# SamsungLabs/fcaf3d

Measured on AMD Instinct MI355X. Metric: scenes/sec fwd+bwd, ScanNet 100k-pt 2cm voxels, 1/2/4/8 MI355X, higher is better.
Workload: dtype f32

## Files before the change

### fcaf3d_amd/csrc/conv.hip

```cpp
#include "fc_common.h"
#include "../../include/fcaf3d_hip.h"
#ifdef FC_TRACE
__device__ unsigned long long* g_trace_buf_lds;
__device__ int g_trace_cap_lds;
extern "C" int fc_debug_trace_lds(unsigned long long* buf, int cap) {
  FC_HIP(hipMemcpyToSymbol(HIP_SYMBOL(g_trace_buf_lds), &buf, sizeof(buf)));
  FC_HIP(hipMemcpyToSymbol(HIP_SYMBOL(g_trace_cap_lds), &cap, sizeof(cap)));
  return FC_OK;
}
#define TR_BUF g_trace_buf_lds
#define TR_CAP g_trace_cap_lds
#endif
#include "fc_trace.h"

typedef float f32x16 __attribute__((ext_vector_type(16)));
typedef float f32x2 __attribute__((ext_vector_type(2)));
typedef float f32x4 __attribute__((ext_vector_type(4)));

__device__ __attribute__((aligned(16))) float g_zero_row[64];

__device__ int g_fc_prio;
extern "C" int fc_debug_set_prio(int mode) {
  FC_HIP(hipMemcpyToSymbol(HIP_SYMBOL(g_fc_prio), &mode, sizeof(mode)));
  return FC_OK;
// ... 1220 lines not shown
    else if (r.bm == 128) FC_TILE(128, 64, 2);
    else if (r.bn == 128) launch_conv_fp32<64, 128, 2>(r, a, grid);
    else launch_conv_fp32<64, 64, 2>(r, a, grid);
#undef FC_TILE
  }
  FC_CHECK_LAUNCH();
  return FC_OK;
}
#undef FC_LAUNCH
#undef FC_LAUNCH_EPI

extern "C" {

int fc_conv_fwd_route(int64_t n_in, int64_t n_out, int K, int Cin, int Cout, int flags, int table_kind, int64_t live_tiles, int* out) {
  if (!out || n_in < 0 || n_out < 0 || K < 1 || Cin < 1 || Cout < 1) return FC_EINVAL;
  const ConvRoute r = conv_route({n_in, n_out, K, Cin, Cout}, flags, table_kind, live_tiles, route_env());
  const int f[16] = {r.family, r.bm, r.bn, r.wm, r.S, r.wsrc, r.mode, r.buf, r.epi, (int)r.grid[0], (int)r.grid[1], (int)r.grid[2]};
  for (int i = 0; i < 16; ++i) out[i] = f[i];
  return r.family == FC_FAM_INVALID ? FC_EINVAL : FC_OK;
}

int64_t fc_conv_fwd_ws_bytes(int64_t n_out, int K, int Cin, int Cout, int flags) {
  const ConvRoute r = conv_route({n_out, n_out, K, Cin, Cout}, flags, FC_TABLE_DENSE, 0, route_env());
  return r.S > 1 ? (int64_t)r.S * n_out * Cout * (int64_t)sizeof(float) : 0;
}

int64_t fc_conv_fwd_pairs_ws_bytes(int64_t n_out, int K, int Cout) {
  return (int64_t)K * n_out * Cout * (int64_t)sizeof(float);
}

int64_t fc_conv_stats_blocks(int64_t n_out, int K, int Cin, int Cout, int flags, int pairs) {
  if (n_out < 1) return 0;
  const ConvRoute r = conv_route({n_out, n_out, K, Cin, Cout}, flags, pairs ? FC_TABLE_PAIRS : FC_TABLE_DENSE, 0, route_env());
  if (r.epi == FC_EPI_NONE) return 0;
  return r.epi == FC_EPI_SUM ? fc_cdiv(n_out, fc_stat_rb(n_out)) : fc_cdiv(n_out, r.bm);
}

static int conv_impl(const float* in, const float* W, const int* nbr, const int* out_index, const int* cnt, const int* pos, float* out,
                     int64_t n_in, int64_t n_out, int K, int Cin, int Cout, int64_t live_tiles, int flags, void* ws, int64_t ws_bytes,
                     hipStream_t stream, const X6Epi* epi) {
  AmaxHintScope hint_scope;
  if (n_in < 0 || n_out < 0 || K < 1 || Cin < 1 || Cout < 1) return FC_EINVAL;
  if (n_out == 0 && !cnt) return epi ? FC_EINVAL : FC_OK;
  if (out_index && !nbr) return FC_EINVAL;
  const int table = cnt ? FC_TABLE_PAIRS : out_index ? FC_TABLE_SORTED : nbr ? FC_TABLE_DENSE : FC_TABLE_NONE;
  const ConvRoute r = conv_route({n_in, n_out, K, Cin, Cout}, flags, table | (epi ? FC_TABLE_STATS : 0), live_tiles, route_env());
  if (r.family == FC_FAM_INVALID) return FC_EINVAL;
  if (n_out == 0) return FC_OK;
  ConvArgs a = {in, W, nbr, out_index, cnt, out, n_out, K, Cin, Cout, {}, stream};
  if (r.family == FC_FAM_STEM || r.family == FC_FAM_FMA) return launch_conv(r, a);
  const bool parts = cnt || r.S > 1;
  if (parts && ws_bytes < (int64_t)r.S * n_out * Cout * (int64_t)sizeof(float)) return FC_EWS;
  if (parts) a.dst = (float*)ws;
  if (epi && r.epi == FC_EPI_KERNEL) a.epi = *epi;
  int rc = FC_OK;
  if (r.mode == FC_MODE_H3) rc = operand_amax(in, n_in * (int64_t)Cin, 0, stream, &a.epi.amax_in);
  if (rc == FC_OK) rc = launch_conv(r, a);
  if (rc != FC_OK || !parts) return rc;
  const int rb = fc_stat_rb(n_out);
  const dim3 sgrid((unsigned)fc_cdiv(n_out, rb), Cout / 64);
  if (cnt && epi) k_sum_pairs_stats<<<sgrid, 256, 0, stream>>>(a.dst, pos, out, n_out, K, Cout, rb, *epi);
  else if (cnt) k_sum_pairs<<<(unsigned)fc_cdiv(n_out * (Cout / 4), 256), 256, 0, stream>>>(a.dst, pos, out, n_out, K, Cout);
  else if (epi) k_sum_parts_stats<<<sgrid, 256, 0, stream>>>(a.dst, out, n_out, Cout, r.S, rb, *epi);
  else k_sum_parts<<<(unsigned)fc_cdiv(n_out * Cout / 4, 256), 256, 0, stream>>>(a.dst, out, n_out * Cout / 4, r.S);
  FC_CHECK_LAUNCH();
  return FC_OK;
}

static int conv_pairs_impl(const float* in, const float* W, const int* pair_in, const int* pair_cnt, const int* pair_pos, float* out,
                           int64_t n_in, int64_t n_out, int K, int Cin, int Cout, int64_t live_tiles, int flags, void* ws,
                           int64_t ws_bytes, hipStream_t stream, const X6Epi* epi) {
  if (!pair_in || !pair_cnt || !pair_pos || K > 65535) return FC_EINVAL;
  return conv_impl(in, W, pair_in, nullptr, pair_cnt, pair_pos, out, n_in, n_out, K, Cin, Cout, live_tiles, flags, ws, ws_bytes, stream, epi);
}

static X6Epi stats_epi(float* stats, const float* bn_x = nullptr, const float* mean = nullptr, const float* var = nullptr, const float* gamma = nullptr,
                       const float* beta = nullptr, float eps = 0.f, int act = 0, const float* add = nullptr, const float* bn_y = nullptr) {
  return {stats, bn_x, mean, var, gamma, beta, eps, act, add, bn_y, nullptr};
}

int fc_conv_fwd(const float* in, const float* W, const int* nbr, const int* out_index, float* out, int64_t n_in,
                int64_t n_out, int K, int Cin, int Cout, int flags, void* ws, int64_t ws_bytes, hipStream_t stream) {
  return conv_impl(in, W, nbr, out_index, nullptr, nullptr, out, n_in, n_out, K, Cin, Cout, 0, flags, ws, ws_bytes, stream, nullptr);
}

int fc_conv_fwd_stats(const float* in, const float* W, const int* nbr, const int* out_index, float* out, int64_t n_in,
                      int64_t n_out, int K, int Cin, int Cout, int flags, void* ws, int64_t ws_bytes, float* stats,
                      hipStream_t stream) {
  const X6Epi e = stats_epi(stats);
  return conv_impl(in, W, nbr, out_index, nullptr, nullptr, out, n_in, n_out, K, Cin, Cout, 0, flags, ws, ws_bytes, stream, stats ? &e : nullptr);
}

int fc_conv_fwd_bn_bwd_stats(const float* in, const float* W, const int* nbr, const int* out_index, float* out, int64_t n_in,
                             int64_t n_out, int K, int Cin, int Cout, int flags, void* ws, int64_t ws_bytes, float* stats,
                             const float* bn_x, const float* mean, const float* var, const float* gamma, const float* beta, float eps,
                             int act, const float* add, const float* bn_y, hipStream_t stream) {
  if (!stats || !bn_x || !mean || !var || act < 0 || act > 2) return FC_EINVAL;
  const X6Epi e = stats_epi(stats, bn_x, mean, var, gamma, beta, eps, act, add, bn_y);
  return conv_impl(in, W, nbr, out_index, nullptr, nullptr, out, n_in, n_out, K, Cin, Cout, 0, flags, ws, ws_bytes, stream, &e);
}

int fc_conv_fwd_pairs_tiles(const float* in, const float* W, const int* pair_in, const int* pair_cnt, const int* pair_pos,
                            float* out, int64_t n_in, int64_t n_out, int K, int Cin, int Cout, int64_t live_tiles, int flags,
                            void* ws, int64_t ws_bytes, hipStream_t stream) {
  return conv_pairs_impl(in, W, pair_in, pair_cnt, pair_pos, out, n_in, n_out, K, Cin, Cout, live_tiles, flags, ws, ws_bytes, stream, nullptr);
}

int fc_conv_fwd_pairs_tiles_stats(const float* in, const float* W, const int* pair_in, const int* pair_cnt, const int* pair_pos,
                                  float* out, int64_t n_in, int64_t n_out, int K, int Cin, int Cout, int64_t live_tiles, int flags,
                                  void* ws, int64_t ws_bytes, float* stats, hipStream_t stream) {
  const X6Epi e = stats_epi(stats);
  return conv_pairs_impl(in, W, pair_in, pair_cnt, pair_pos, out, n_in, n_out, K, Cin, Cout, live_tiles, flags, ws, ws_bytes, stream,
                         stats ? &e : nullptr);
}

int fc_conv_fwd_pairs_tiles_bn_bwd_stats(const float* in, const float* W, const int* pair_in, const int* pair_cnt, const int* pair_pos,
                                         float* out, int64_t n_in, int64_t n_out, int K, int Cin, int Cout, int64_t live_tiles, int flags,
                                         void* ws, int64_t ws_bytes, float* stats, const float* bn_x, const float* mean,
                                         const float* var, const float* gamma, const float* beta, float eps, int act,
                                         const float* add, const float* bn_y, hipStream_t stream) {
  if (!stats || !bn_x || !mean || !var || act < 0 || act > 2) return FC_EINVAL;
  const X6Epi e = stats_epi(stats, bn_x, mean, var, gamma, beta, eps, act, add, bn_y);
  return conv_pairs_impl(in, W, pair_in, pair_cnt, pair_pos, out, n_in, n_out, K, Cin, Cout, live_tiles, flags, ws, ws_bytes, stream, &e);
}

int fc_conv_fwd_pairs(const float* in, const float* W, const int* pair_in, const int* pair_cnt, const int* pair_pos,
                      float* out, int64_t n_in, int64_t n_out, int K, int Cin, int Cout, int flags, void* ws,
                      int64_t ws_bytes, hipStream_t stream) {
  return fc_conv_fwd_pairs_tiles(in, W, pair_in, pair_cnt, pair_pos, out, n_in, n_out, K, Cin, Cout, 0, flags, ws, ws_bytes, stream);
}

int64_t fc_x6_weight_image_bytes(int K, int R, int C) { return (int64_t)K * R * C * 6; }

int fc_x6_weight_image(const float* W, void* img, int K, int R, int C, int transposed, hipStream_t stream) {
  if (K < 1 || R < 32 || C < 64 || R % 32 != 0 || C % 64 != 0) return FC_EINVAL;
  const int64_t total = (int64_t)K * (R / 32) * (C / 64) * 256;
  const unsigned nb = (unsigned)fc_cdiv(total, 256);
  if (split_mode() == 2) {
    FC_HIP(hipMemsetAsync((char*)img + 4 * X6_IMG_AMAX_WORD, 0, FC_AMAX_SLOT_BYTES, stream));
    k_x6_weight_image<3><<<nb, 256, 0, stream>>>(W, (u32x4*)img, K, R, C, transposed);
    k_x6_weight_image<2><<<nb, 256, 0, stream>>>(W, (u32x4*)img, K, R, C, transposed);
  } else {
    k_x6_weight_image<0><<<nb, 256, 0, stream>>>(W, (u32x4*)img, K, R, C, transposed);
  }
  FC_CHECK_LAUNCH();
  return FC_OK;
}

int fc_x6_weight_images(const int64_t* desc, int n, int64_t total_blocks, hipStream_t stream) {
  if (!desc || n < 1 || total_blocks < 1 || total_blocks > 0x7fffffffll) return FC_EINVAL;
  const long long* d = reinterpret_cast<const long long*>(desc);
  if (split_mode() == 2) {
    k_x6_weight_images<4><<<(unsigned)fc_cdiv(n, 4), 256, 0, stream>>>(d, n);
    k_x6_weight_images<3><<<(unsigned)total_blocks, 256, 0, stream>>>(d, n);
    k_x6_weight_images<2><<<(unsigned)total_blocks, 256, 0, stream>>>(d, n);
  } else {
    k_x6_weight_images<0><<<(unsigned)total_blocks, 256, 0, stream>>>(d, n);
  }
  FC_CHECK_LAUNCH();
  return FC_OK;
}

}

template <int BMc, int BNc, bool HAS_NBR, int BKR, bool PAIRS>
__global__ __launch_bounds__(256, 2) void k_wgrad_mfma(const float* __restrict__ in, const float* __restrict__ gout,
                                                    const int* __restrict__ nbr, const int* __restrict__ row_index,
                                                    const int* __restrict__ cnt,
                                                    float* __restrict__ part, int64_t n_out, int K, int Cin, int Cout,
                                                    int64_t rows_per_split) {
  constexpr int TM = BMc / 64, TN = BNc / 64;
  constexpr int AR = BMc * BKR / 1024, GR = BNc * BKR / 1024;
  __shared__ __attribute__((aligned(16))) float As[BKR * BMc];
  __shared__ __attribute__((aligned(16))) float Gs[BKR * BNc];
  const int tid = threadIdx.x, lane = tid & 63, wave = tid >> 6;
  const int wr = wave >> 1, wc = wave & 1;
  const int r = lane & 31, h = lane >> 5;
  const int tiles_n = Cout / BNc, tiles_m = Cin / BMc;
  int y = blockIdx.y;
  const int tn = y % tiles_n; y /= tiles_n;
  const int tm = y % tiles_m; y /= tiles_m;
  const int k = y;
  const int ci0 = tm * BMc, co0 = tn * BNc;
  int64_t total = n_out;
  if (PAIRS) {
    total = cnt[k];
    rows_per_split = ((total + gridDim.x - 1) / gridDim.x + BKR - 1) / BKR * BKR;
  }
  const int64_t r_begin = (int64_t)blockIdx.x * rows_per_split;
  int64_t r_end = r_begin + rows_per_split;
  if (r_end > total) r_end = total;

  f32x16 acc[TM][TN];
#pragma unroll
  for (int i = 0; i < TM; ++i)
#pragma unroll
    for (int j = 0; j < TN; ++j)
#pragma unroll
      for (int e = 0; e < 16; ++e) acc[i][j][e] = 0.f;

  f32x4 av[AR], gv[GR];
  auto load_chunk = [&](int64_t rb) {
    int src[AR];
#pragma unroll
    for (int i = 0; i < AR; ++i) {
      int lin = tid + 256 * i;
      int rr = lin / (BMc / 4);
      int64_t row = rb + rr;
      int64_t rc = row < r_end ? row : r_end - 1;
      int t = HAS_NBR ? nbr[(int64_t)k * n_out + rc] : (int)rc;
      src[i] = row < r_end ? t : -1;
    }
#pragma unroll
    for (int i = 0; i < GR; ++i) {
      int lin = tid + 256 * i;
      int rr = lin / (BNc / 4), c4 = lin % (BNc / 4);
      int64_t row = rb + rr;
      int64_t rc = row < r_end ? row : r_end - 1;
      if (PAIRS) rc = row_index[(int64_t)k * n_out + rc];
      const float* gp = row < r_end ? gout + rc * Cout + co0 + c4 * 4 : g_zero_row + (c4 & 15) * 4;
      gv[i] = *reinterpret_cast<const f32x4*>(gp);
    }
#pragma unroll
    for (int i = 0; i < AR; ++i) {
      int lin = tid + 256 * i;
      int c4 = lin % (BMc / 4);
      const float* ap = src[i] < 0 ? g_zero_row + (c4 & 15) * 4 : in + (int64_t)src[i] * Cin + ci0 + c4 * 4;
      av[i] = *reinterpret_cast<const f32x4*>(ap);
    }
  };
  if (r_begin < r_end) load_chunk(r_begin);
  for (int64_t rb = r_begin; rb < r_end; rb += BKR) {
    __syncthreads();
#pragma unroll
    for (int i = 0; i < AR; ++i) {
      int lin = tid + 256 * i;
      int rr = lin / (BMc / 4), c4 = lin % (BMc / 4);
      *reinterpret_cast<f32x4*>(&As[rr * BMc + c4 * 4]) = av[i];
    }
#pragma unroll
    for (int i = 0; i < GR; ++i) {
      int lin = tid + 256 * i;
      int rr = lin / (BNc / 4), c4 = lin % (BNc / 4);
      *reinterpret_cast<f32x4*>(&Gs[rr * BNc + c4 * 4]) = gv[i];
    }
    __syncthreads();
    if (rb + BKR < r_end) load_chunk(rb + BKR);
#pragma unroll
    for (int q = 0; q < BKR / 8; ++q) {
      float a[TM][4], b[TN][4];
#pragma unroll
      for (int e = 0; e < 4; ++e) {
#pragma unroll
        for (int i = 0; i < TM; ++i) a[i][e] = As[(8 * q + 4 * h + e) * BMc + wr * (BMc / 2) + i * 32 + r];
#pragma unroll
        for (int j = 0; j < TN; ++j) b[j][e] = Gs[(8 * q + 4 * h + e) * BNc + wc * (BNc / 2) + j * 32 + r];
      }
#pragma unroll
      for (int e = 0; e < 4; ++e)
#pragma unroll
        for (int i = 0; i < TM; ++i)
#pragma unroll
          for (int j = 0; j < TN; ++j) acc[i][j] = __builtin_amdgcn_mfma_f32_32x32x2f32(a[i][e], b[j][e], acc[i][j], 0, 0, 0);
    }
  }
  float* dst = part + ((int64_t)blockIdx.x * K + k) * Cin * Cout;
#pragma unroll
  for (int i = 0; i < TM; ++i)
#pragma unroll
    for (int j = 0; j < TN; ++j)
#pragma unroll
      for (int e = 0; e < 16; ++e) {
        int row = ci0 + wr * (BMc / 2) + i * 32 + (e & 3) + 8 * (e >> 2) + 4 * h;
        int col = co0 + wc * (BNc / 2) + j * 32 + r;
        dst[(int64_t)row * Cout + col] = acc[i][j][e];
      }
}

template <int BNc, bool HAS_NBR, bool PAIRS>
__global__ __launch_bounds__(256, 3) void k_wgrad_mfma_p(const float* __restrict__ in, const float* __restrict__ gout,
                                                          const int* __restrict__ nbr, const int* __restrict__ row_index,
                                                          const int* __restrict__ cnt, float* __restrict__ part,
                                                          int64_t n_out, int K, int Cin, int Cout, int64_t rows_per_split) {
  constexpr int BMc = 64, BKR = 32;
  constexpr int TN = BNc / 64;
  constexpr int AR = 2, GR = BNc * BKR / 1024;
  __shared__ __attribute__((aligned(16))) float As[BKR * BMc];
  __shared__ __attribute__((aligned(16))) float Gs[BKR * BNc];
  const int tid = threadIdx.x, lane = tid & 63, wave = tid >> 6;
  const int wr = wave >> 1, wc = wave & 1;
  const int r = lane & 31, h = lane >> 5;
  const int tiles_n = Cout / BNc, tiles_m = Cin / BMc;
  int y = blockIdx.y;
  const int tn = y % tiles_n; y /= tiles_n;
  const int tm = y % tiles_m; y /= tiles_m;
  const int k = y;
  const int ci0 = tm * BMc, co0 = tn * BNc;
  int64_t total = n_out;
  if (PAIRS) {
    total = cnt[k];
    rows_per_split = ((total + gridDim.x - 1) / gridDim.x + BKR - 1) / BKR * BKR;
  }
  const int64_t r_begin = (int64_t)blockIdx.x * rows_per_split;
  int64_t r_end = r_begin + rows_per_split;
  if (r_end > total) r_end = total;

  f32x16 acc[TN];
// ... 443 lines not shown
```

### fcaf3d_amd/csrc/conv_x6.h

```cpp
#pragma once

typedef __bf16 bf16x8 __attribute__((ext_vector_type(8)));
typedef unsigned int u32x4 __attribute__((ext_vector_type(4)));
typedef unsigned int u32x2 __attribute__((ext_vector_type(2)));

typedef __bf16 x6_bf16x2 __attribute__((ext_vector_type(2)));
typedef float x6_f32x2 __attribute__((ext_vector_type(2)));
__device__ __forceinline__ unsigned x6_hi2(unsigned u0, unsigned u1) { return __builtin_amdgcn_perm(u1, u0, 0x07060302u); }
__device__ __forceinline__ unsigned x6_rn2(float x0, float x1) {
  const x6_f32x2 v = {x0, x1};
  return __builtin_bit_cast(unsigned, __builtin_convertvector(v, x6_bf16x2));
}
__device__ __forceinline__ void x6_split2(float x0, float x1, unsigned& p0, unsigned& p1, unsigned& p2) {
  p0 = x6_rn2(x0, x1);
  const float r0 = x0 - __uint_as_float(p0 << 16), r1 = x1 - __uint_as_float(p0 & 0xffff0000u);
  p1 = x6_rn2(r0, r1);
  const float s0 = r0 - __uint_as_float(p1 << 16), s1 = r1 - __uint_as_float(p1 & 0xffff0000u);
  p2 = x6_rn2(s0, s1);
}

typedef _Float16 x6_f16x2 __attribute__((ext_vector_type(2)));
typedef _Float16 f16x8 __attribute__((ext_vector_type(8)));
#define X6_IMG_AMAX_WORD 2048
__device__ __forceinline__ float h3_scale(unsigned amax_bits) {
// ... 20 lines not shown
__device__ __forceinline__ void h3_split2s(float x0, float x1, float s, unsigned& p0, unsigned& p1) {
  h3_split2(x0 * s, x1 * s, p0, p1);
}

__device__ __forceinline__ int x6_bslot(int c, int plane, int chunk) {
  const int row = (c & 1) * 32 + (c >> 1);
  return (plane * 64 + row) * 4 + (chunk ^ ((row >> 2) & 3));
}
#define X6_GROUP_U16 (3 * 64 * 4)

__device__ __forceinline__ void x6_weight_image_unit(const float* __restrict__ W, u32x4* __restrict__ img, int64_t t, int R, int C,
                                                     int transposed) {
  const int chunk = (int)(t & 3), c = (int)((t >> 2) & 63);
  const int64_t blk = t >> 8;
  const int g = (int)(blk % (C / 64));
  const int slab = (int)((blk / (C / 64)) % (R / 32));
  const int k = (int)(blk / ((int64_t)(C / 64) * (R / 32)));
  const int col = g * 64 + c, r0 = slab * 32 + chunk * 8;
  const float* Wk = W + (int64_t)k * R * C;
  float x[8];
#pragma unroll
  for (int e = 0; e < 8; ++e) x[e] = transposed ? Wk[(int64_t)col * R + r0 + e] : Wk[(int64_t)(r0 + e) * C + col];
  unsigned p[3][4];
#pragma unroll
  for (int e = 0; e < 4; ++e) x6_split2(x[2 * e], x[2 * e + 1], p[0][e], p[1][e], p[2][e]);
#pragma unroll
  for (int pl = 0; pl < 3; ++pl) {
    u32x4 v = {p[pl][0], p[pl][1], p[pl][2], p[pl][3]};
    img[blk * X6_GROUP_U16 + x6_bslot(c, pl, chunk)] = v;
  }
}

__device__ __forceinline__ void h3_weight_image_unit(const float* __restrict__ W, u32x4* __restrict__ img, int64_t t, int R, int C,
                                                     int transposed, float sw) {
  const int chunk = (int)(t & 3), c = (int)((t >> 2) & 63);
  const int64_t blk = t >> 8;
  const int g = (int)(blk % (C / 64));
  const int slab = (int)((blk / (C / 64)) % (R / 32));
  const int k = (int)(blk / ((int64_t)(C / 64) * (R / 32)));
  const int col = g * 64 + c, r0 = slab * 32 + chunk * 8;
  const float* Wk = W + (int64_t)k * R * C;
  float x[8];
#pragma unroll
  for (int e = 0; e < 8; ++e) x[e] = transposed ? Wk[(int64_t)col * R + r0 + e] : Wk[(int64_t)(r0 + e) * C + col];
  unsigned p[2][4];
#pragma unroll
  for (int e = 0; e < 4; ++e) h3_split2s(x[2 * e], x[2 * e + 1], sw, p[0][e], p[1][e]);
#pragma unroll
  for (int pl = 0; pl < 2; ++pl) {
    u32x4 v = {p[pl][0], p[pl][1], p[pl][2], p[pl][3]};
    img[blk * X6_GROUP_U16 + x6_bslot(c, pl, chunk)] = v;
  }
}
__device__ __forceinline__ unsigned h3_weight_unit_amax(const float* __restrict__ W, int64_t t, int R, int C, int transposed) {
  const int chunk = (int)(t & 3), c = (int)((t >> 2) & 63);
  const int64_t blk = t >> 8;
  const int g = (int)(blk % (C / 64));
  const int slab = (int)((blk / (C / 64)) % (R / 32));
  const int k = (int)(blk / ((int64_t)(C / 64) * (R / 32)));
  const int col = g * 64 + c, r0 = slab * 32 + chunk * 8;
  const float* Wk = W + (int64_t)k * R * C;
  unsigned m = 0u;
#pragma unroll
  for (int e = 0; e < 8; ++e) {
    const unsigned u = __float_as_uint(transposed ? Wk[(int64_t)col * R + r0 + e] : Wk[(int64_t)(r0 + e) * C + col]) & 0x7fffffffu;
    m = (u > m && u < 0x7f800000u) ? u : m;
  }
  return m;
}
__device__ __forceinline__ void h3_block_amax(unsigned m, unsigned* __restrict__ slot) {
#pragma unroll
  for (int off = 32; off > 0; off >>= 1) { const unsigned o = (unsigned)__shfl_xor((int)m, off, 64); m = o > m ? o : m; }
  if ((threadIdx.x & 63) == 0) {
    unsigned* w = slot + (blockIdx.x & (FC_AMAX_SUB - 1)) * FC_AMAX_STRIDE;
    if (m > __hip_atomic_load(w, __ATOMIC_RELAXED, __HIP_MEMORY_SCOPE_AGENT)) atomicMax(w, m);
  }
}

template <int MODE>
__global__ void k_x6_weight_image(const float* __restrict__ W, u32x4* __restrict__ img, int K, int R, int C, int transposed) {
  const int64_t t = (int64_t)blockIdx.x * blockDim.x + threadIdx.x;
  const bool live = t < (int64_t)K * (R / 32) * (C / 64) * 256;
  if (MODE == 3) { h3_block_amax(live ? h3_weight_unit_amax(W, t, R, C, transposed) : 0u, reinterpret_cast<unsigned*>(img) + X6_IMG_AMAX_WORD); return; }
  if (MODE == 2) {
    const float sw = h3_scale(fc_amax_read(reinterpret_cast<const unsigned*>(img) + X6_IMG_AMAX_WORD));
    if (live) h3_weight_image_unit(W, img, t, R, C, transposed, sw);
    return;
  }
  if (live) x6_weight_image_unit(W, img, t, R, C, transposed);
}
#if 0
__global__ void k_x6_weight_image(const float* __restrict__ W, u32x4* __restrict__ img, int K, int R, int C, int transposed) {
  const int64_t t = (int64_t)blockIdx.x * blockDim.x + threadIdx.x;
  if (t < (int64_t)K * (R / 32) * (C / 64) * 256) x6_weight_image_unit(W, img, t, R, C, transposed);
}
#endif

#define X6_IMG_LD 65
__device__ __forceinline__ void h3_weight_image_unit_lds(const float* __restrict__ W, u32x4* __restrict__ img, int64_t blk, int R, int C,
                                                         int transposed, float sw, float* __restrict__ tile ) {
  const int g = (int)(blk % (C / 64));
  const int slab = (int)((blk / (C / 64)) % (R / 32));
  const int k = (int)(blk / ((int64_t)(C / 64) * (R / 32)));
  const float* Wk = W + (int64_t)k * R * C;
  const int tid = threadIdx.x;
  if (!transposed) {
#pragma unroll
    for (int p = 0; p < 2; ++p) {
      const int r = p * 16 + (tid >> 4), c4 = (tid & 15) * 4;
      const float4 v = *reinterpret_cast<const float4*>(Wk + (int64_t)(slab * 32 + r) * C + g * 64 + c4);
      tile[r * X6_IMG_LD + c4] = v.x; tile[r * X6_IMG_LD + c4 + 1] = v.y; tile[r * X6_IMG_LD + c4 + 2] = v.z; tile[r * X6_IMG_LD + c4 + 3] = v.w;
    }
  } else {
#pragma unroll
    for (int p = 0; p < 2; ++p) {
      const int c = p * 32 + (tid >> 3), r4 = (tid & 7) * 4;
      const float4 v = *reinterpret_cast<const float4*>(Wk + (int64_t)(g * 64 + c) * R + slab * 32 + r4);
      tile[r4 * X6_IMG_LD + c] = v.x; tile[(r4 + 1) * X6_IMG_LD + c] = v.y; tile[(r4 + 2) * X6_IMG_LD + c] = v.z; tile[(r4 + 3) * X6_IMG_LD + c] = v.w;
    }
  }
  __syncthreads();
  const int chunk = tid & 3, c = (tid >> 2) & 63;
  unsigned p[2][4];
#pragma unroll
  for (int e = 0; e < 4; ++e)
    h3_split2s(tile[(chunk * 8 + 2 * e) * X6_IMG_LD + c], tile[(chunk * 8 + 2 * e + 1) * X6_IMG_LD + c], sw, p[0][e], p[1][e]);
#pragma unroll
  for (int pl = 0; pl < 2; ++pl) {
    u32x4 v = {p[pl][0], p[pl][1], p[pl][2], p[pl][3]};
    img[blk * X6_GROUP_U16 + x6_bslot(c, pl, chunk)] = v;
  }
}

template <int MODE>
__global__ __launch_bounds__(256) void k_x6_weight_images(const long long* __restrict__ desc, int n) {
  if (MODE == 4) {
    const int e = blockIdx.x * (blockDim.x / 64) + (threadIdx.x >> 6), l = threadIdx.x & 63;
    if (e < n && l < FC_AMAX_SUB) reinterpret_cast<unsigned*>(desc[8 * e + 1])[X6_IMG_AMAX_WORD + l * FC_AMAX_STRIDE] = 0u;
    return;
  }
  int lo = 0, hi = n - 1;
  const long long b = blockIdx.x;
  while (lo < hi) {
    const int mid = (lo + hi + 1) >> 1;
    if (desc[8 * mid + 6] <= b) lo = mid; else hi = mid - 1;
  }
  const long long* d = desc + 8 * lo;
  const int K = (int)d[2], R = (int)d[3], C = (int)d[4];
  const int64_t t = (b - d[6]) * 256 + threadIdx.x;
  const bool live = t < (int64_t)K * (R / 32) * (C / 64) * 256;
  const float* W = reinterpret_cast<const float*>(d[0]);
  u32x4* img = reinterpret_cast<u32x4*>(d[1]);
  const bool vec = (reinterpret_cast<uintptr_t>(W) & 15) == 0;
  if (MODE == 3) {
    if (d[7]) return;
    unsigned m = 0u;
    if (live && vec) {
      const float4* w4 = reinterpret_cast<const float4*>(W + t * 8);
      const float4 x0 = w4[0], x1 = w4[1];
      const float xs[8] = {x0.x, x0.y, x0.z, x0.w, x1.x, x1.y, x1.z, x1.w};
#pragma unroll
      for (int e = 0; e < 8; ++e) {
        const unsigned v = __float_as_uint(xs[e]) & 0x7fffffffu;
        m = (v > m && v < 0x7f800000u) ? v : m;
      }
    } else if (live) {
      m = h3_weight_unit_amax(W, t, R, C, (int)d[5]);
    }
    h3_block_amax(m, reinterpret_cast<unsigned*>(img) + X6_IMG_AMAX_WORD);
    return;
  }
  if (MODE == 2) {
    __shared__ float tile[32 * X6_IMG_LD];
    const unsigned* slot = d[7] ? reinterpret_cast<const unsigned*>(d[7]) + X6_IMG_AMAX_WORD : reinterpret_cast<const unsigned*>(img) + X6_IMG_AMAX_WORD;
    const unsigned am = fc_amax_read(slot);
    if (d[7] && b == d[6] && threadIdx.x == 0) reinterpret_cast<unsigned*>(img)[X6_IMG_AMAX_WORD] = am;
    if (!live) return;
    if (vec) h3_weight_image_unit_lds(W, img, t >> 8, R, C, (int)d[5], h3_scale(am), tile);
    else h3_weight_image_unit(W, img, t, R, C, (int)d[5], h3_scale(am));
    return;
  }
  if (live) x6_weight_image_unit(W, img, t, R, C, (int)d[5]);
}

#define X6_MFMA(A, B, C) __builtin_amdgcn_mfma_f32_32x32x16_bf16(__builtin_bit_cast(bf16x8, A), __builtin_bit_cast(bf16x8, B), C, 0, 0, 0)
#define H3_MFMA(A, B, C) __builtin_amdgcn_mfma_f32_32x32x16_f16(__builtin_bit_cast(f16x8, A), __builtin_bit_cast(f16x8, B), C, 0, 0, 0)

struct X6Epi {
  float* stats;
  const float* bn_x;
  const float* mean;
  const float* var;
  const float* gamma;
  const float* beta;
  float eps;
  int act;
  const float* add;
  const float* bn_y;
  const unsigned* amax_in;
};

__device__ __forceinline__ void x6_epi_terms(bool bwd, float v, float xv, float mu, float is, float ga, float be, int act, bool from_y,
                                             float yv, float& t1, float& t2) {
  if (!bwd) {
    t1 = v;
    t2 = v * v;
  } else {
    float d = 1.f;
    if (from_y) {
      if (act == 1) d = yv > 0.f ? 1.f : 0.f;
      else if (act == 2) d = yv > 0.f ? 1.f : yv + 1.f;
    } else {
      const float pre = fmaf((xv - mu) * is, ga, be);
      if (act == 1) d = pre > 0.f ? 1.f : 0.f;
      else if (act == 2) d = pre > 0.f ? 1.f : expf(pre);
    }
    const float g = v * d;
    t1 = g;
    t2 = g * ((xv - mu) * is);
  }
}

template <int BM, int BN, bool HAS_NBR, int WM, int BSRC, int MODE = 0, bool BUF = false>
__global__ __launch_bounds__(256, BM == 256 ? 2 : (BN == 64 ? 4 : 3)) void k_conv_x6(
    const float* __restrict__ in, const float* __restrict__ W, const int* __restrict__ nbr,
    const int* __restrict__ out_index, const int* __restrict__ cnt, float* __restrict__ out, int64_t n_out, int K, int Cin,
    int Cout, X6Epi epi) {
  float* __restrict__ stats = epi.stats;
  constexpr int WN = 4 / WM;
  constexpr int TM = BM / (32 * WM), TN = BN / (32 * WN);
  constexpr int RW = BM / WM;
  constexpr int AR = BM / 32;
  constexpr int CPT = BN / 64;
  constexpr int BU = 3 * BN / 64;
  constexpr bool WT = BSRC == 1;
  constexpr bool FAST = MODE == 1;
  constexpr bool H3 = MODE == 2 && BSRC == 2;
  constexpr int NPL = H3 ? 2 : 3;
  constexpr int GU = NPL * 64 * 4;
  __shared__ u32x4 As[NPL * BM * 4];
  __shared__ u32x4 Bs[(BN / 64) * GU];
  __shared__ unsigned int kmask_s;

  const int tid = threadIdx.x, lane = tid & 63, wave = tid >> 6;
  const int wr = WM == 4 ? wave : wave >> 1, wc = WM == 4 ? 0 : wave & 1;
  const int r = lane & 31, h = lane >> 5;
  const int bgrp = TN == 2 ? wc : 0;
  int64_t bx = blockIdx.x;
  const int n0 = blockIdx.y * BN;
  int S = gridDim.z, z = blockIdx.z;
  int kbase = 0;
  if (cnt) {
    if (gridDim.z == 1 && K > 1) {
      int k = 0;
      for (; k < K - 1; ++k) {
        const int64_t t = ((int64_t)cnt[k] + BM - 1) / BM;
        if (bx < t) break;
        bx -= t;
      }
      z = k;
    }
    const int64_t stride = n_out;
    n_out = cnt[z];
    if (bx * BM >= n_out) return;
    nbr += (int64_t)z * stride;
    if (BSRC == 2) kbase = z; else W += (int64_t)z * Cin * Cout;
    out += (int64_t)z * stride * Cout;
    K = 1; S = 1; z = 0;
  }
  const int64_t m0 = bx * BM;
  const int a_c4 = tid & 7, a_r = tid >> 3;
  float h3_sa = 1.f, h3_inv = 1.f;
  if (H3) {
    h3_sa = h3_scale(fc_amax_read(epi.amax_in));
    h3_inv = h3_unscale(h3_sa, h3_scale(fc_amax_read(reinterpret_cast<const unsigned*>(W) + X6_IMG_AMAX_WORD)));
  }

  f32x16 acc[TM][TN];
#pragma unroll
  for (int i = 0; i < TM; ++i)
#pragma unroll
    for (int j = 0; j < TN; ++j)
#pragma unroll
      for (int e = 0; e < 16; ++e) acc[i][j][e] = 0.f;

  unsigned int kmask;
  {
    if (tid == 0) kmask_s = 0u;
    __syncthreads();
    if (tid < BM) {
      unsigned int mk = 0u;
      int64_t row = m0 + tid;
      if (row < n_out) {
        if (HAS_NBR) {
          for (int k = z; k < K; k += S)
            if (nbr[(int64_t)k * n_out + row] >= 0) mk |= 1u << k;
        } else {
          mk = 1u;
        }
      }
      for (int off = 32; off > 0; off >>= 1) mk |= __shfl_xor(mk, off, 64);
      if (lane == 0 && mk) atomicOr(&kmask_s, mk);
    }
    __syncthreads();
    kmask = BUF ? (unsigned int)__builtin_amdgcn_readfirstlane((int)kmask_s) : kmask_s;
  }
  constexpr bool buf = BUF && BSRC == 2;
  constexpr unsigned X6_DEAD = 0x80000000u;

  if (kmask) {
    const int nst = __popc(kmask) * (Cin / 32);
    unsigned int rem = kmask;
    int lk = __ffs(rem) - 1;
    rem &= rem - 1;
    int lnk = rem ? __ffs(rem) - 1 : lk;
    if (rem) rem &= rem - 1;
    int lc0 = 0;
    bool sw = false;
    constexpr bool fast = FAST && BSRC == 2;
    f32x4 av[AR];
    f32x4 bw[2 * CPT];
    float bf[8][CPT];
    u32x4 bi[BU];
    int vcur[AR], vnxt[AR];
    const int rows_here = (int)((n_out - m0) < BM ? (n_out - m0) : BM);
    const __amdgpu_buffer_rsrc_t rn = __builtin_amdgcn_make_buffer_rsrc(const_cast<int*>(nbr), 0, 0x7fffffff, 0x00020000);
    unsigned irow[AR];
#pragma unroll
    for (int i = 0; i < AR; ++i) irow[i] = (a_r + 32 * i < rows_here ? (unsigned)(m0 + a_r + 32 * i) : 0u) * 4u;
    auto fetch_idx = [&](int kk, int (&v)[AR]) {
#pragma unroll
      for (int i = 0; i < AR; ++i) {
        if (BUF && BSRC == 2 && HAS_NBR) {
          v[i] = (int)__builtin_amdgcn_raw_buffer_load_b32(rn, (int)irow[i], (int)((unsigned)kk * (unsigned)n_out * 4u), 0);
          continue;
// ... 313 lines not shown
```

### fcaf3d_amd/executor.py

```python
import os
import struct

import numpy as np
import torch

from . import _lib as L
from . import functional as Fn
from . import nn as MEnn

ENABLED = os.environ.get('FC_EXEC', '1') != '0'
PROBE = None
TRUSTED = None
KEEP_STATE = False


def _layouts():
    names, fields = {}, {}
    for block in L.parse_enums():
        names.update(block)
        *members, end = block
        op = names.get('OP_' + end[:-len('_END')]) if end.endswith('_END') else None
        if op is not None:
            fields[op] = {n[len(end) - 3:].lower().removesuffix('_p1'): (block[n], n.endswith('_P1')) for n in members}
    return {k: v for k, v in names.items() if k.startswith('OP_') or k in ('OPW', 'MAPW', 'ROW_OP', 'ROW_STREAM')}, fields


_NAMES, FIELDS = _layouts()
globals().update(_NAMES)


def word(op, field):
    return FIELDS[op][field][0]


ALIGN = 256
S_MAIN, S_HEAD, S_WGRAD = 0, 1, 2
EV_FORK, EV_HEAD_DONE, EV_W0, EV_W1, EV_WEND, EV_BWD0, EV_HB = 0, 8, 9, 10, 11, 12, 16


def _f(x):
    return struct.unpack('<q', struct.pack('<d', float(x)))[0]


def supported(det):
    bb, nh = det.backbone, det.neck_with_head
    if not (ENABLED and Fn.X6 and not (Fn.FLAGS & Fn.CONV_FMA) and Fn.STEM_COL and Fn.DGRAD_WT):
        return False
    if getattr(bb.BLOCK, 'expansion', 1) != 1 or det.spatial_sort:
        return False
    if 1 + nh.n_reg_outs + nh.n_classes > 64 or bb.conv1[0].in_channels != 3:
        return False
    return type(nh).forward_single is _FORWARD_SINGLE and type(nh).forward is _NECK_FORWARD


_FORWARD_SINGLE = _NECK_FORWARD = None


class NetProgram:
    def __init__(self, det, training, wgrad_async, head_overlap, tail0=False, keep_state=None):
        self.det = det
        self.tail0 = tail0
        self.keep_state = bool(KEEP_STATE if keep_state is None else keep_state)
        self.training = training
        self.wgrad_async = wgrad_async and training
        bb, nh = det.backbone, det.neck_with_head
        self.nl = min(bb.n_outs, 4)
        self.head_overlap = head_overlap and self.nl > 1
        self.dev = next(det.parameters()).device
        self.ops_f, self.ops_b = [], []
        self.n_addr = 0
        self.static = []
        self.arena = {'f': [], 'b': []}
        self.alias = []
        self.dyn = {}
        self.dim_names = {}
        self.map_names = {}
        self.grad_refs = []
        self.keep = []
        self.relu_outs = []
        self.pool_arg = None
        self.out_idx = None
        self.gout_idx = self.x0_idx = ()
        self.in_sums = None
        self.small = []
        self._pready = {}
        self._params = [p for p in det.parameters() if p.requires_grad]
        self._goff, off = {}, 0
        flat = getattr(self._params[0], '_fc_flat', None)
        self.flat = flat[0] if flat is not None else None
        for p in self._params:
            if self.flat is not None:
                assert p._fc_flat[0] is self.flat
                self._goff[id(p)] = p._fc_flat[1]
            else:
                self._goff[id(p)] = off
                off += -(-p.numel() // 64) * 64
        self._gtotal = self.flat.n if self.flat is not None else off
        self._sig = self.signature(det)
        self._build_weights()
        self._build(_Emitter(self))
        self._finalise()

    @staticmethod
    def signature(det):
        from .flat import GENERATION
        return GENERATION[0]

    def _new(self):
        self.n_addr += 1
        return self.n_addr - 1

    def D(self, name):
        if name not in self.dim_names:
            self.dim_names[name] = len(self.dim_names)
        return self.dim_names[name]

    def M(self, name):
        if name not in self.map_names:
            self.map_names[name] = len(self.map_names)
        return self.map_names[name]

    def T(self, rows, cols, arena='f', elem=4, extra=0):
        i = self._new()
        self.arena[arena].append((i, self.D(rows), cols * elem, extra))
        return i

    def S(self, tensor):
        i = self._new()
        self.static.append((i, tensor.data_ptr()))
        self.keep.append(tensor)
        return i

    def SA(self, address):
        i = self._new()
        self.static.append((i, int(address)))
        return i

    def DY(self, name):
        if name not in self.dyn:
            self.dyn[name] = self._new()
        return self.dyn[name]

    def AL(self, parent, off_dim, cols, elem=4):
        i = self._new()
        self.alias.append((i, parent, self.D(off_dim), cols * elem))
        return i

    def G(self, p):
        i = self._new()
        self.grad_refs.append((i, self._goff[id(p)]))
        return i

    def emit(self, lst, op, stream, **fields):
        row = [0] * OPW
        row[ROW_OP], row[ROW_STREAM] = op, stream
        self.patch(row, **fields)
        lst.append(row)

    @staticmethod
    def patch(row, **fields):
        layout = FIELDS[row[ROW_OP]]
        for k, v in fields.items():
            if k not in layout:
                raise KeyError(f'operator {row[ROW_OP]} has no field {k!r}')
            w, p1 = layout[k]
            row[w] = v + 1 if p1 else v

    def _build_weights(self):
        holder = self.det.__dict__.get('_exec_weights')
        if holder is None or holder.sig != self._sig:
            holder = self.det.__dict__['_exec_weights'] = _Weights(self.det, self.dev, self._sig)
        self.w = holder
        self.packed, self.gent_w, self.gents, self.images, self.ncol = holder.packed, holder.gent_w, holder.gents, holder.images, holder.ncol

    @property
    def weights_fresh(self):
        return self.w.fresh

    @weights_fresh.setter
    def weights_fresh(self, v):
        self.w.fresh = v

    def refresh_weights(self):
        self.w.refresh()

    def IMG(self, w, transposed):
        v = self.w.img_of[w.data_ptr()]
        assert v is not None and v[1 if transposed else 0] is not None, 'no split-bf16 image for this kernel shape'
        return self.S(v[1 if transposed else 0])

    def _build(self, em):
        bb, nh = self.det.backbone, self.det.neck_with_head
        x = em.stem(bb.conv1[0], bb.conv1[1])
        levels = []
        for li in range(1, self.nl + 1):
            x = em.level(li, getattr(bb, f'layer{li}'), x)
            levels.append(x)
        self.out_idx = (self.T('Nall', 1), self.T('Nall', nh.n_reg_outs), self.T('Nall', nh.n_classes), self.T('Nall', 1))
        if self.training:
            em.tape.append(lambda: em.flush_small(S_MAIN))
            self.gout_idx = (self.DY('g_cent'), self.DY('g_bbox'), self.DY('g_cls'))
        for i in range(self.nl - 1, -1, -1):
            if i < self.nl - 1:
                x = em.up(i, getattr(nh, f'up_block_{i + 1}'), x, levels[i])
            if i == 0 and self.tail0:
                self.x0_idx = x
                if self.training:
                    em.grads.arrive(x[0], self.DY('g_x0'), *x[1:], S_MAIN)
            else:
                em.head(i, getattr(nh, f'out_block_{i}'), x)
        if self.head_overlap:
            em.sync(self.ops_f, S_HEAD, S_MAIN, EV_HEAD_DONE)
        em.backward()

    def _finalise(self):
        self.ops_f = np.ascontiguousarray(np.asarray(self.ops_f, dtype=np.int64).reshape(-1, OPW))
        self.ops_b = np.ascontiguousarray(np.asarray(self.ops_b, dtype=np.int64).reshape(-1, OPW)) if self.ops_b else np.zeros((0, OPW), np.int64)
        self.addr0 = np.zeros(self.n_addr, dtype=np.int64)
        for i, a in self.static:
            self.addr0[i] = a

        def columns(table, width):
            return tuple(np.ascontiguousarray(np.array(table, dtype=np.int64).reshape(-1, width).T))
        self._ar = {k: columns(a, 4) for k, a in self.arena.items()}
        self._al = columns(self.alias, 4)
        self._gr = columns([(i, 4 * off) for i, off in self.grad_refs], 2)
        self.n_dims, self.n_maps = len(self.dim_names), len(self.map_names)
        self._ws = [None, None, None]
        self._need = np.zeros(3, dtype=np.int64)
        self._cfg = np.array([Fn.BN_SMALL_ELEMS, Fn.FLAGS, 0, 0], dtype=np.int64)
        self.n_conv_f = int((self.ops_f[:, ROW_OP] == OP_CONV).sum())
        self.n_conv_b = int((self.ops_b[:, ROW_OP] == OP_CONV).sum()) if len(self.ops_b) else 0
        self.n_amax = int((self.ops_f[:, ROW_OP] == OP_AMAX).sum()) + (int((self.ops_b[:, ROW_OP] == OP_AMAX).sum()) if len(self.ops_b) else 0)
        self._anchor = torch.zeros(1, device=self.dev, requires_grad=True)
        if self.training:
            n = len(self.small)
            self._small = np.zeros((2 * n, 8), dtype=np.int64)
            self._small_goff = np.zeros(2 * n, dtype=np.int64)
            self._small_in = None
            for k, (src, nseg, C, w, b) in enumerate(self.small):
                for h, p in ((0, b), (1, w)):
                    r = 2 * k + h
                    self._small[r, 2], self._small[r, 3], self._small[r, 4] = C, 1, 2 * C
                    self._small_goff[r] = self._goff[id(p)] * 4
                    if src is not None:
                        self._small[r, 0] = src + 4 * C * h
                    else:
                        self._small_in = (2 * k, C)

    def _fill_arena(self, addr, dims, which, base):
        idx, di, bpr, ext = self._ar[which]
        if len(idx) == 0:
            return
        sizes = (dims[di] * bpr + ext + (ALIGN - 1)) // ALIGN * ALIGN
        offs = np.cumsum(sizes) - sizes
        addr[idx] = base + offs

    def _arena_bytes(self, dims, which):
        idx, di, bpr, ext = self._ar[which]
        return int(((dims[di] * bpr + ext + (ALIGN - 1)) // ALIGN * ALIGN).sum()) + ALIGN

    def bind(self, x, batch_size, backward):
        nl = self.nl
        cm0 = x.cmap
        dims = np.zeros(self.n_dims, dtype=np.int64)
        maps = np.zeros((self.n_maps, MAPW), dtype=np.int64)
        dn, mn, N = self.dim_names, self.map_names, _Names

        def setd(k, v):
            if k in dn:
                dims[dn[k]] = v
        m1 = cm0.strided(2)
        m2 = m1.strided(2)
        maps[mn['stem']] = cm0.kernel_map(m1, 3).desc(conv=False)
        maps[mn['pool']] = m1.kernel_map(m2, 2).desc(conv=False)
        kms = {}
        setd('n0', cm0.n); setd('n1', m1.n); setd('n2', m2.n); setd('B', batch_size); setd('one', 1)
        prev, lv = m2, []
        for li in range(1, nl + 1):
            mi = prev.strided(2)
            kms[N.down(li)], kms[N.ds(li)], kms[N.same(li)] = prev.kernel_map(mi, 3), prev.kernel_map(mi, 1), mi.kernel_map(mi, 3)
            for k in (N.down(li), N.ds(li), N.same(li)):
                maps[mn[k]] = kms[k].desc(True, backward)
            setd(N.rows(li), mi.n)
            lv.append(mi)
            prev = mi
        xm = lv[-1]
        head_maps = [xm]
        dyn = {}
        for i in range(nl - 2, -1, -1):
            g = xm.generate()
            u, rows, swapped = lv[i].union(g)
            if not swapped or u is not g:
                return None
            kms[N.gsame(i)] = g.kernel_map(g, 3)
            maps[mn[N.gsame(i)]] = kms[N.gsame(i)].desc(True, backward)
            setd(N.gen(i), g.n)
            dyn[N.union(i)] = rows
            xm = g
            head_maps.append(g)
        head_maps = head_maps[::-1]
        off = 0
        for i, cm in enumerate(head_maps):
            if i == 0 and self.tail0:
                continue
            setd(N.off(i), off)
            off += cm.n
        setd('Nall', off)
        st = dict(dims=dims, maps=maps, dyn=dyn, head_maps=head_maps, x=x, seg1=m1.coords, n_all=off)
        if PROBE is not None:
            from .sparse import _rec
            st['pairs'] = {mn[k]: _rec(km._pairs[3].sum() if km._pairs is not None else (km.nbr >= 0).sum()) for k, km in kms.items()}
            PROBE.append(dict(pairs=st['pairs'], nf=self.n_conv_f, nb=self.n_conv_b, na=self.n_amax))
        return st

    def _streams(self):
        dev = self.dev
        nh = self.det.neck_with_head
        main = L.stream()
        head = nh._head_stream(dev).cuda_stream if self.head_overlap else main
        wg = Fn.wgrad_stream(dev).cuda_stream if self.wgrad_async else main
        return np.array([main, head, wg], dtype=np.int64)

    def _run(self, ops, addr, st, begin=0, end=None, size_only=False):
        streams = self._streams()
        self._cfg[2] = 1 if 'pairs' in st else 0
        self._cfg[3] = 1 if size_only else 0
        end = len(ops) if end is None else end
        while True:
            ws = np.array([w.data_ptr() if w is not None else 0 for w in self._ws], dtype=np.int64)
            wsb = np.array([w.numel() if w is not None else 0 for w in self._ws], dtype=np.int64)
            rc = L.lib().fc_exec(ops.ctypes.data, begin, end, addr.ctypes.data, st['dims'].ctypes.data, st['maps'].ctypes.data,
                                 streams.ctypes.data, ws.ctypes.data, wsb.ctypes.data, self._need.ctypes.data, self._cfg.ctypes.data)
            if rc == -2:
                for i in range(3):
                    if self._need[i] > wsb[i]:
                        self._ws[i] = torch.empty(int(self._need[i] * 5 // 4) + (1 << 20), dtype=torch.uint8, device=self.dev)
                continue
            if rc != 0:
                raise RuntimeError(f'fc_exec failed: {"invalid argument" if rc == -1 else "hipError %d" % rc}')
            return

    def decisions(self, st):
        assert self.keep_state, 'this program does not store the stem\'s normalised output: build it under executor.KEEP_STATE'
        relu = [(self._view(st, *t) > 0).cpu() for t in self.relu_outs]
        return relu, self._view(st, *self.pool_arg, torch.int32).cpu()

    def _view(self, st, idx, rows, C, dtype=torch.float32):
        fa, n = st['fa'], int(st['dims'][self.dim_names[rows]])
        o = int(st['addr'][idx] - fa.data_ptr())
        return fa[o:o + n * C * 4].view(dtype).view(n, C)

    def forward(self, st):
        trusted = (TRUSTED is not None and TRUSTED.w is self.w) or (not self.training and getattr(self.det, 'static_weights', False))
        if not (self.weights_fresh and trusted):
            self.refresh_weights()
        ev = self.images.event
        if ev is not None:
            torch.cuda.current_stream().wait_event(ev)
        if self.training:
            return _NetFn.apply(self._anchor, self, st)
        return self._forward(st)

    def _forward(self, st):
        dims = st['dims']
        fa = torch.empty(self._arena_bytes(dims, 'f'), dtype=torch.uint8, device=self.dev)
        addr = self.addr0.copy()
        base = (fa.data_ptr() + ALIGN - 1) // ALIGN * ALIGN
        self._fill_arena(addr, dims, 'f', base)
        addr[self.dyn['x0']] = st['x'].F.data_ptr()
        addr[self.dyn['seg1']] = st['seg1'].data_ptr()
        for k, t in st['dyn'].items():
            addr[self.dyn[k]] = t.data_ptr()
        ai, ap, ad, ab = self._al
        fwd_alias = addr[ap] != 0
        addr[ai[fwd_alias]] = addr[ap[fwd_alias]] + dims[ad[fwd_alias]] * ab[fwd_alias]
        st['fa'], st['addr'] = fa, addr
        self._run(self.ops_f, addr, st)
        nh = self.det.neck_with_head
        outs = [self._view(st, idx, 'Nall', c) for idx, c in zip(self.out_idx, (1, nh.n_reg_outs, nh.n_classes, 1))]
        if self.tail0:
            outs.append(self._view(st, *self.x0_idx))
        return tuple(outs)

    def _backward(self, st, g_cent, g_bbox, g_cls, g_x0=None):
        dims, addr = st['dims'], st['addr']
        n = st['n_all']
        nh = self.det.neck_with_head
        gs = []
        for g, c in zip((g_cent, g_bbox, g_cls), (1, nh.n_reg_outs, nh.n_classes)):
            gs.append(g.contiguous() if g is not None else torch.zeros((n, c), dtype=torch.float32, device=self.dev))
        if self.tail0:
            t, rows, C = self.x0_idx
            n0 = int(dims[self.dim_names[rows]])
            g_x0 = g_x0.contiguous() if g_x0 is not None else torch.zeros((n0, C), dtype=torch.float32, device=self.dev)
            gs.append(g_x0)
        ba = torch.empty(self._arena_bytes(dims, 'b'), dtype=torch.uint8, device=self.dev)
        base = (ba.data_ptr() + ALIGN - 1) // ALIGN * ALIGN
        self._fill_arena(addr, dims, 'b', base)
        for k, g in zip(('g_cent', 'g_bbox', 'g_cls', 'g_x0'), gs):
            addr[self.dyn[k]] = g.data_ptr()
        ai, ap, ad, ab = self._al
        addr[ai] = addr[ap] + dims[ad] * ab
        own = self._own_params()
        pre = [(p, p.grad) for p in own if p.grad is not None]
        aliased = self.flat is not None and any(g.data_ptr() == self.flat.grad_view(p).data_ptr() for p, g in pre)
        accum = bool(pre) and (self.flat is None or aliased or len(pre) > 16)
        if self.flat is not None and not accum:
            gbuf = self.flat.grad
        else:
            gbuf = torch.zeros(self._gtotal, dtype=torch.float32, device=self.dev)
        gi, go = self._gr
        addr[gi] = gbuf.data_ptr() + go
        desc = self._small.copy()
        desc[:, 1] = gbuf.data_ptr() + self._small_goff
        r, C = self._small_in
        B = int(dims[self.dim_names['B']])
        desc[r, 0], desc[r + 1, 0] = addr[self.in_sums], addr[self.in_sums] + 4 * C
        desc[r:r + 2, 3] = B
        desc_dev = L.upload(desc, self.dev)
        addr[self.dyn['small_desc']] = desc_dev.data_ptr()
        gv = self._grad_views(gbuf)
        if not accum:
            for p in own:
                p.grad = gv[id(p)]
        from . import dist as D
        av = D.ACTIVE
        if av is not None and av.buckets and av.flat is self.flat and self.flat is not None and not accum and not self.tail0:
            pos = 0
            self._run(self.ops_b, addr, st, size_only=True)
            for upto in self._bucket_ready(av):
                if upto > pos:
                    self._run(self.ops_b, addr, st, pos, upto)
                    pos = upto
                av.launch_next()
            if pos < len(self.ops_b):
                self._run(self.ops_b, addr, st, pos, len(self.ops_b))
        else:
            self._run(self.ops_b, addr, st)
        if accum:
            for p in own:
                if p.grad is None:
                    p.grad = gv[id(p)]
                else:
                    p.grad.add_(gv[id(p)])
        else:
            for p, g0 in pre:
                gv[id(p)].add_(g0)
            if self.flat is not None and not self.tail0:
                self.flat.complete = True
        st['ba'] = ba

    def _own_params(self):
        c = getattr(self, '_own', None)
        if c is None:
            c = self._own = [p for p in self._params if id(p) in self._pready]
        return c

    def _bucket_ready(self, av):
        key = id(av)
        c = getattr(self, '_br', None)
        if c is None or c[0] != key:
            out, run = [], 0
            for b in av.buckets:
                run = max(run, max(self._pready[id(p)] for p in b))
                out.append(run)
            c = self._br = (key, out)
        return c[1]

    def _grad_views(self, gbuf):
        key = gbuf.data_ptr()
        cache = getattr(self, '_gv', None)
        if cache is None or cache[0] != key:
            views = {id(p): gbuf[self._goff[id(p)]:self._goff[id(p)] + p.numel()].view(p.shape) for p in self._params}
            cache = self._gv = (key, views, gbuf)
        return cache[1]


class _Names:
    rows, down, ds, same = 'L{}'.format, 'down{}'.format, 'ds{}'.format, 'same{}'.format
    gen, gsame, off, union = 'g{}'.format, 'gsame{}'.format, 'off{}'.format, 'rows{}'.format


class _Grads:

    def __init__(self, em):
        self.em = em
        self.full = {}
        self.second = {}
        self.behind = {}
        self.src = {}

    def _add(self, t, g, rows, cols, stream):
        em, dst = self.em, self.full[t]
        em.p.emit(em.Bk, OP_ADD, stream, dst=dst, src=g, n=em.p.D(rows), c=cols)
        self.src.pop(dst, None)
        em.amax_of.pop(dst, None)

    def arrive(self, t, g, rows, cols, stream):
        if t not in self.full:
            self.full[t] = g
        elif Fn.BN_FUSE and t not in self.second:
            self.second[t] = (g, rows, cols, stream)
        else:
            self.own(t)
            self._add(t, g, rows, cols, stream)

    def take(self, t, rows, cols, pair=False):
        if t in self.behind:
            g, lvl = self.behind.pop(t)
            self.em.join(lvl)
            self.arrive(t, g, rows, cols, S_MAIN)
        if pair:
            return self.full[t], (self.second.pop(t)[0] if t in self.second else None)
        return self.own(t)

    def own(self, t):
        if t in self.second:
            self._add(t, *self.second.pop(t))
        return self.full[t]

    def deliver(self, t, lvl):
        self.behind[t] = (self.own(t), lvl)
        del self.full[t]


class _Emitter:

    AMAX_SLOTS = 1024
    AMAX_SLOT_BYTES = 2048

# ... 384 lines not shown
```

Before: 511.9.

## Run stem ops before waiting on weight images and batch amax reduction

Replaces the per-unit weight amax kernel with one that processes 8 units per block, reduces with wave shuffles and uses a single guarded atomicMax per block. This cuts atomic traffic and launch granularity. The executor also finds the first forward op that touches weight buffers and runs the ops before it before waiting on the image-build event, so stem work overlaps weight image preparation. The cost is added complexity: _run must support range and size_only arguments, and the earlier ops must truly not depend on the image buffers.

```diff
diff --git a/fcaf3d_amd/csrc/conv.hip b/fcaf3d_amd/csrc/conv.hip
--- a/fcaf3d_amd/csrc/conv.hip
+++ b/fcaf3d_amd/csrc/conv.hip
@@ -1396,7 +1396,7 @@
   const long long* d = reinterpret_cast<const long long*>(desc);
   if (split_mode() == 2) {
     k_x6_weight_images<4><<<(unsigned)fc_cdiv(n, 4), 256, 0, stream>>>(d, n);
-    k_x6_weight_images<3><<<(unsigned)total_blocks, 256, 0, stream>>>(d, n);
+    k_x6_weight_amax<<<(unsigned)fc_cdiv(total_blocks, X6_AMAX_UNITS), 256, 0, stream>>>(d, n, total_blocks);
     k_x6_weight_images<2><<<(unsigned)total_blocks, 256, 0, stream>>>(d, n);
   } else {
     k_x6_weight_images<0><<<(unsigned)total_blocks, 256, 0, stream>>>(d, n);
diff --git a/fcaf3d_amd/csrc/conv_x6.h b/fcaf3d_amd/csrc/conv_x6.h
--- a/fcaf3d_amd/csrc/conv_x6.h
+++ b/fcaf3d_amd/csrc/conv_x6.h
@@ -196,24 +196,6 @@
   const float* W = reinterpret_cast<const float*>(d[0]);
   u32x4* img = reinterpret_cast<u32x4*>(d[1]);
   const bool vec = (reinterpret_cast<uintptr_t>(W) & 15) == 0;
-  if (MODE == 3) {
-    if (d[7]) return;
-    unsigned m = 0u;
-    if (live && vec) {
-      const float4* w4 = reinterpret_cast<const float4*>(W + t * 8);
-      const float4 x0 = w4[0], x1 = w4[1];
-      const float xs[8] = {x0.x, x0.y, x0.z, x0.w, x1.x, x1.y, x1.z, x1.w};
-#pragma unroll
-      for (int e = 0; e < 8; ++e) {
-        const unsigned v = __float_as_uint(xs[e]) & 0x7fffffffu;
-        m = (v > m && v < 0x7f800000u) ? v : m;
-      }
-    } else if (live) {
-      m = h3_weight_unit_amax(W, t, R, C, (int)d[5]);
-    }
-    h3_block_amax(m, reinterpret_cast<unsigned*>(img) + X6_IMG_AMAX_WORD);
-    return;
-  }
   if (MODE == 2) {
     __shared__ float tile[32 * X6_IMG_LD];
     const unsigned* slot = d[7] ? reinterpret_cast<const unsigned*>(d[7]) + X6_IMG_AMAX_WORD : reinterpret_cast<const unsigned*>(img) + X6_IMG_AMAX_WORD;
@@ -225,6 +207,63 @@
     return;
   }
   if (live) x6_weight_image_unit(W, img, t, R, C, (int)d[5]);
+}
+
+#define X6_AMAX_UNITS 8
+__global__ __launch_bounds__(256) void k_x6_weight_amax(const long long* __restrict__ desc, int n, long long total_blocks) {
+  __shared__ unsigned wm[4];
+  long long u = (long long)blockIdx.x * X6_AMAX_UNITS;
+  const long long u_end = u + X6_AMAX_UNITS < total_blocks ? u + X6_AMAX_UNITS : total_blocks;
+  int lo = 0, hi = n - 1;
+  while (lo < hi) {
+    const int mid = (lo + hi + 1) >> 1;
+    if (desc[8 * mid + 6] <= u) lo = mid; else hi = mid - 1;
+  }
+  for (int e = lo; e < n && u < u_end; ++e) {
+    const long long* d = desc + 8 * e;
+    const long long first = d[6], next = e + 1 < n ? d[8 + 6] : total_blocks;
+    const long long stop = next < u_end ? next : u_end;
+    const int R = (int)d[3], C = (int)d[4];
+    const long long live = first + (long long)d[2] * (R / 32) * (C / 64);
+    const long long lim = live < stop ? live : stop;
+    if (!d[7] && first <= u && u < lim) {
+      const float* W = reinterpret_cast<const float*>(d[0]);
+      unsigned m = 0u;
+      if ((reinterpret_cast<uintptr_t>(W) & 15) == 0) {
+        const f32x4* w4 = reinterpret_cast<const f32x4*>(W) + (u - first) * 512;
+        const int n4 = (int)(lim - u) * 512;
+        for (int i = threadIdx.x; i < n4; i += 4 * 256) {
+          f32x4 v[4];
+#pragma unroll
+          for (int q = 0; q < 4; ++q) v[q] = i + q * 256 < n4 ? w4[i + q * 256] : f32x4{0.f, 0.f, 0.f, 0.f};
+#pragma unroll
+          for (int q = 0; q < 4; ++q)
+#pragma unroll
+            for (int j = 0; j < 4; ++j) {
+              const unsigned x = __float_as_uint(v[q][j]) & 0x7fffffffu;
+              m = (x > m && x < 0x7f800000u) ? x : m;
+            }
+        }
+      } else {
+        for (long long uu = u; uu < lim; ++uu) {
+          const unsigned x = h3_weight_unit_amax(W, (uu - first) * 256 + threadIdx.x, R, C, (int)d[5]);
+          m = x > m ? x : m;
+        }
+      }
+#pragma unroll
+      for (int off = 32; off > 0; off >>= 1) { const unsigned o = (unsigned)__shfl_xor((int)m, off, 64); m = o > m ? o : m; }
+      if ((threadIdx.x & 63) == 0) wm[threadIdx.x >> 6] = m;
+      __syncthreads();
+      if (threadIdx.x == 0) {
+        unsigned b = wm[0];
+        for (int w = 1; w < 4; ++w) b = wm[w] > b ? wm[w] : b;
+        unsigned* s = reinterpret_cast<unsigned*>(d[1]) + X6_IMG_AMAX_WORD + (blockIdx.x & (FC_AMAX_SUB - 1)) * FC_AMAX_STRIDE;
+        if (b > __hip_atomic_load(s, __ATOMIC_RELAXED, __HIP_MEMORY_SCOPE_AGENT)) atomicMax(s, b);
+      }
+      __syncthreads();
+    }
+    u = stop;
+  }
 }
 
 #define X6_MFMA(A, B, C) __builtin_amdgcn_mfma_f32_32x32x16_bf16(__builtin_bit_cast(bf16x8, A), __builtin_bit_cast(bf16x8, B), C, 0, 0, 0)
diff --git a/fcaf3d_amd/executor.py b/fcaf3d_amd/executor.py
--- a/fcaf3d_amd/executor.py
+++ b/fcaf3d_amd/executor.py
@@ -12,6 +12,7 @@
 PROBE = None
 TRUSTED = None
 KEEP_STATE = False
+STEM_UNDER_IMAGES = True
 
 
 def _layouts():
@@ -233,6 +234,7 @@
         self.n_conv_b = int((self.ops_b[:, ROW_OP] == OP_CONV).sum()) if len(self.ops_b) else 0
         self.n_amax = int((self.ops_f[:, ROW_OP] == OP_AMAX).sum()) + (int((self.ops_b[:, ROW_OP] == OP_AMAX).sum()) if len(self.ops_b) else 0)
         self._anchor = torch.zeros(1, device=self.dev, requires_grad=True)
+        self.first_image_op = self._first_image_op()
         if self.training:
             n = len(self.small)
             self._small = np.zeros((2 * n, 8), dtype=np.int64)
@@ -247,6 +249,20 @@
                         self._small[r, 0] = src + 4 * C * h
                     else:
                         self._small_in = (2 * k, C)
+
+    def weight_spans(self):
+        w = self.w
+        bufs = [w.packed] + list(w.gent_w) + ([w.images.buf] if w.images.n else [])
+        return [(t.data_ptr(), t.data_ptr() + t.numel() * t.element_size()) for t in bufs]
+
+    def _first_image_op(self):
+        spans = self.weight_spans()
+        hot = {i for i, a in self.static if any(lo <= a < hi for lo, hi in spans)}
+        for r, row in enumerate(self.ops_f):
+            layout = FIELDS.get(int(row[ROW_OP]), {})
+            if any(int(row[w]) - (1 if p1 else 0) in hot for w, p1 in layout.values()):
+                return r
+        return len(self.ops_f)
 
     def _fill_arena(self, addr, dims, which, base):
         idx, di, bpr, ext = self._ar[which]
@@ -356,8 +372,12 @@
         if not (self.weights_fresh and trusted):
             self.refresh_weights()
         ev = self.images.event
+        st['images_event'] = None
         if ev is not None:
-            torch.cuda.current_stream().wait_event(ev)
+            if STEM_UNDER_IMAGES and self.first_image_op > 0:
+                st['images_event'] = ev
+            else:
+                torch.cuda.current_stream().wait_event(ev)
         if self.training:
             return _NetFn.apply(self._anchor, self, st)
         return self._forward(st)
@@ -376,7 +396,15 @@
         fwd_alias = addr[ap] != 0
         addr[ai[fwd_alias]] = addr[ap[fwd_alias]] + dims[ad[fwd_alias]] * ab[fwd_alias]
         st['fa'], st['addr'] = fa, addr
-        self._run(self.ops_f, addr, st)
+        ev = st.pop('images_event', None)
+        if ev is None:
+            self._run(self.ops_f, addr, st)
+        else:
+            k = self.first_image_op
+            self._run(self.ops_f, addr, st, size_only=True)
+            self._run(self.ops_f, addr, st, 0, k)
+            torch.cuda.current_stream().wait_event(ev)
+            self._run(self.ops_f, addr, st, k, len(self.ops_f))
         nh = self.det.neck_with_head
         outs = [self._view(st, idx, 'Nall', c) for idx, c in zip(self.out_idx, (1, nh.n_reg_outs, nh.n_classes, 1))]
         if self.tail0:
```

Result: no change. 516.6 (median of 6 runs) (+0.9%).
